# KTH-RPL/neural_graph_mapping

Hardware: AMD Instinct MI355X
Metric: ray-samples/sec (train step: fwd+loss+bwd+Adam, 4096 rays x 128 samples per GPU) (higher is better)
Workload: dtype f32 via 3xbf16 split, fp32 accumulate (hidden-layer matrix products, forward and backward); everything else f32; 1 GPU; M1: 8 fields x 512 rays x (64 coarse + 64 depth-guided) samples per GPU, Fourier(64,raw)+2x64 MLP, nrgbd compositing, NRGBD intrinsics; fields_per_gpu=8, rays_per_field=512, samples_per_ray=128, ranks_seen=1, spin_up_steps=200, jitter=in-kernel Philox, launch=hipGraph replay

## Files before the change

### include/ngm_hip.h

```cpp
#ifndef NGM_HIP_H
#define NGM_HIP_H

#include <stdint.h>

#ifdef __cplusplus
extern "C" {
#endif

#define NGM_ABI_VERSION 11
#define NGM_MAX_LAYERS 4
#define NGM_NUM_LOSS_SUMS 16

enum ngm_status {
  NGM_OK = 0,
  NGM_E_INVALID = -1,
  NGM_E_UNSUPPORTED = -2,
  NGM_E_WORKSPACE = -3,
  NGM_E_HIP = -4
};

enum ngm_encoding { NGM_ENC_NONE = 0, NGM_ENC_FOURIER = 1, NGM_ENC_NERF = 2, NGM_ENC_PERMUTO = 3, NGM_ENC_TRIPLANE = 4 };
enum ngm_triplane_mode { NGM_TRI_SUM = 0, NGM_TRI_PRODUCT = 1, NGM_TRI_CONCAT = 2 };
enum ngm_skip_mode { NGM_SKIP_NO = 0, NGM_SKIP_ADD = 1, NGM_SKIP_CONCAT = 2 };
enum ngm_matmul_mode { NGM_MATMUL_F32 = 0, NGM_MATMUL_BF16X3 = 1, NGM_MATMUL_AUTO = 2 };
// ... 327 lines not shown
                            int64_t max_verts, int64_t* faces, int64_t max_faces, void* workspace,
                            int64_t workspace_bytes, void* stream);
int ngm_marching_cubes_tables(int8_t* tri_table, int32_t* tri_count);

enum ngm_kernel_id {
  NGM_K_RENDER_FWD = 0,
  NGM_K_STASH_BWD = 1,
  NGM_K_FIELD_BWD = 2,
  NGM_K_GRAD_REDUCE = 3,
  NGM_K_ADAM = 4,
  NGM_K_POINTS_FWD = 5,
  NGM_K_COMPOSITE_FWD = 6,
  NGM_K_COMPOSITE_BWD = 7,
  NGM_K_HASH_GRAD = 8,
  NGM_K_HASH_REDUCE = 9,
  NGM_K_LOSS_REDUCE = 10,
  NGM_K_KNN_ASSIGN = 11,
  NGM_K_KNN_EVAL = 12,
  NGM_K_SAMPLER = 13,
  NGM_K_COUNT = 14
};
int ngm_profile_enable(int32_t on);
int ngm_profile_reset(void);
int ngm_profile_read(int32_t kernel_id, double* total_ms, int64_t* launches);

int ngm_debug_phase_cycles(unsigned long long* out528);
int ngm_debug_fwd_phase_cycles(unsigned long long* out528);

int ngm_debug_last_bwd_variant(void);
int ngm_debug_last_matmul(int which);
int ngm_debug_last_fwd_one_tile(void);
int ngm_debug_last_comp_fused(void);
int ngm_debug_disable_fused_comp(int on);
int ngm_debug_stash_mode(int mode);
int ngm_debug_last_stash_mode(void);

#define NGM_MAX_PEERS 8
typedef struct ngm_peer_exchange {
  int32_t world, rank;
  void* mailbox[NGM_MAX_PEERS];
  unsigned long long* seq;
  int32_t* status;
} ngm_peer_exchange;
int64_t ngm_peer_mailbox_bytes(void);
int ngm_peer_alloc(int64_t bytes, void** ptr);
int ngm_peer_free(void* ptr);
int ngm_ipc_export(void* ptr, unsigned char handle[64]);
int ngm_ipc_open(const unsigned char handle[64], void** ptr);
int ngm_ipc_close(void* ptr);
int ngm_loss_exchange(const ngm_peer_exchange* px, float* loss_sums , void* stream);
double ngm_peer_set_timeout(double seconds);

#ifdef __cplusplus
}
#endif
#endif
```

### neural_graph_mapping_amd/_capi.py

```python
import ctypes as C
import os

HERE = os.path.dirname(os.path.abspath(__file__))
LIB_PATH = os.environ.get("NGM_LIB_PATH") or os.path.join(HERE, "lib", "libngm_hip.so")

NGM_MAX_LAYERS = 4
NGM_NUM_LOSS_SUMS = 16
ENC = {"none": 0, "fourier": 1, "nerf": 2, "permuto": 3, "triplane": 4}
TRI = {"sum": 0, "product": 1, "concat": 2}
SCALE = {"no": 0, "unit_ball": 1, "unit_cube": 2}
GEO = {"nrgbd": 0, "occupancy": 1, "density": 2, "neus": 3}
PHOTO = {"l1": 0, "l2": 1, "gaussian_nll": 2}
DEPTH = {"huber": 0, "gaussian_nll": 1, "laplacian_nll": 2}
LS = dict(PHOTO_SUM=0, PHOTO_CNT=1, DEPTH_SUM=2, DEPTH_CNT=3, FS_SUM=4, FS_CNT=5, TSDF_SUM=6,
          TSDF_CNT=7, TERM_SUM=8, TERM_CNT=9, PHOTO_L1_SUM=10)

f32p = C.c_void_p
LArr = C.c_void_p * (NGM_MAX_LAYERS + 1)
SArr = C.c_int64 * (NGM_MAX_LAYERS + 1)


class FieldCfg(C.Structure):
    _fields_ = [("encoding", C.c_int32), ("dim_enc", C.c_int32), ("raw_coords", C.c_int32),
                ("num_octaves", C.c_int32), ("start_octave", C.c_int32), ("num_layers", C.c_int32),
# ... 178 lines not shown
    L.ngm_ipc_close.argtypes = [vp]
    L.ngm_loss_exchange.argtypes = [P(PeerExchange), vp, vp]
    L.ngm_peer_set_timeout.argtypes = [C.c_double]
    L.ngm_peer_set_timeout.restype = C.c_double
    L.ngm_adam_sparse_multi.restype = C.c_int
    L.ngm_step_advance.restype = C.c_int
    L.ngm_field_eval_knn.argtypes = [P(FieldCfg), P(Params), i32, i64, vp, vp, vp, i32, f32, f32, f32, vp, vp, i64, vp]
    L.ngm_field_eval_knn_workspace.argtypes = [i32, i64, i32]
    L.ngm_field_eval_knn_workspace.restype = i64
    L.ngm_render_eval_knn.argtypes = [P(FieldCfg), P(RenderCfg), P(Params), i32, vp, vp, P(Rays), i32, f32, f32, f32, i32,
                                      P(Prediction), vp, i64, vp]
    L.ngm_render_eval_knn.restype = C.c_int
    L.ngm_render_eval_knn_workspace.argtypes = [P(RenderCfg), i32, i32, i32]
    L.ngm_render_eval_knn_workspace.restype = i64
    L.ngm_target_visibility.argtypes = [P(Keyframes), i32, vp, i32, vp, f32, vp, vp, vp]
    L.ngm_target_rays.argtypes = [P(Keyframes), i32, i32, vp, f32, vp, vp, vp, P(TargetOut), vp]
    L.ngm_target_visibility.restype = C.c_int
    L.ngm_target_rays.restype = C.c_int
    L.ngm_target_sv_intersect.argtypes = [i32, i64, vp, vp, f32, vp, vp]
    L.ngm_target_sv_intersect.restype = C.c_int
    L.ngm_target_sv_rays.argtypes = [i32, i32, vp, f32, vp, vp, vp, i32, i32, f32, f32, f32, f32, P(TargetOut), vp]
    L.ngm_target_sv_rays.restype = C.c_int
    L.ngm_target_sample_mv_workspace.argtypes = [i32, i32, i32, i32]
    L.ngm_target_sample_mv_workspace.restype = i64
    L.ngm_target_sample_mv.argtypes = [P(Keyframes), P(TargetSample), P(TargetOut), vp, i64, vp]
    L.ngm_target_sample_mv.restype = C.c_int
    L.ngm_marching_cubes_workspace.argtypes = [i32, i32, i32]
    L.ngm_marching_cubes_workspace.restype = i64
    L.ngm_marching_cubes_count.argtypes = [vp, i32, i32, i32, f32, vp, vp, i64, vp]
    L.ngm_marching_cubes_emit.argtypes = [vp, i32, i32, i32, f32, vp, i64, vp, i64, vp, i64, vp]
    L.ngm_marching_cubes_tables.argtypes = [vp, vp]
    for name in ("ngm_marching_cubes_count", "ngm_marching_cubes_emit", "ngm_marching_cubes_tables"):
        getattr(L, name).restype = C.c_int
    L.ngm_profile_enable.argtypes = [i32]
    L.ngm_profile_read.argtypes = [i32, P(C.c_double), P(i64)]
    for name in ("ngm_profile_enable", "ngm_profile_reset", "ngm_profile_read"):
        getattr(L, name).restype = C.c_int
    for name in ("ngm_sample_rays", "ngm_field_eval_fwd", "ngm_field_eval_bwd", "ngm_composite_fwd",
                 "ngm_composite_bwd", "ngm_render_fwd", "ngm_render_bwd", "ngm_render_bwd_seeded",
                 "ngm_render_read_samples", "ngm_adam_sparse", "ngm_field_eval_knn", "ngm_device_info"):
        getattr(L, name).restype = C.c_int
    _lib = L
    return L


EXPORTED = ["ngm_abi_version", "ngm_last_error", "ngm_device_info", "ngm_permuto_fill_scales", "ngm_sample_rays", "ngm_sample_rays_world", "ngm_sample_rays_weighted",
            "ngm_composite_fwd_packed",
            "ngm_field_eval_fwd", "ngm_encode_fwd", "ngm_encode_bwd", "ngm_encode_bwd_workspace", "ngm_field_eval_bwd", "ngm_field_eval_bwd_workspace",
            "ngm_field_eval_stash_bytes", "ngm_field_eval_fwd_train", "ngm_field_eval_bwd_stash",
            "ngm_composite_fwd", "ngm_composite_bwd", "ngm_render_workspace", "ngm_render_fwd",
            "ngm_render_bwd", "ngm_render_bwd_adam", "ngm_render_bwd_seeded", "ngm_render_bwd_seeded_vars", "ngm_render_read_samples", "ngm_adam_sparse",
            "ngm_field_eval_knn", "ngm_field_eval_knn_workspace", "ngm_render_eval_knn", "ngm_render_eval_knn_workspace", "ngm_adam_sparse_multi", "ngm_step_advance", "ngm_profile_enable", "ngm_profile_reset", "ngm_profile_read",
            "ngm_debug_phase_cycles", "ngm_debug_fwd_phase_cycles", "ngm_debug_last_bwd_variant", "ngm_debug_last_matmul", "ngm_debug_last_fwd_one_tile", "ngm_debug_last_comp_fused", "ngm_debug_disable_fused_comp", "ngm_debug_stash_mode", "ngm_debug_last_stash_mode", "ngm_target_visibility", "ngm_target_rays", "ngm_target_sv_intersect", "ngm_target_sv_rays",
            "ngm_target_sample_mv_workspace", "ngm_target_sample_mv",
            "ngm_render_fwd_counted", "ngm_render_bwd_counted", "ngm_render_bwd_adam_counted",
            "ngm_peer_mailbox_bytes", "ngm_peer_alloc", "ngm_peer_free", "ngm_ipc_export", "ngm_ipc_open", "ngm_ipc_close", "ngm_loss_exchange", "ngm_peer_set_timeout",
            "ngm_marching_cubes_workspace", "ngm_marching_cubes_count", "ngm_marching_cubes_emit", "ngm_marching_cubes_tables"]

NO_GRAD_PARAMS = frozenset({"_encoding.random_shift_per_level"})

KERNEL_IDS = dict(render_fwd=0, stash_bwd=1, field_bwd=2, grad_reduce=3, adam=4, points_fwd=5, composite_fwd=6,
                  composite_bwd=7, hash_grad=8, hash_reduce=9, loss_reduce=10, knn_assign=11, knn_eval=12, sampler=13)


NGM_OK, NGM_E_INVALID, NGM_E_UNSUPPORTED, NGM_E_WORKSPACE, NGM_E_HIP = 0, -1, -2, -3, -4


class NgmError(RuntimeError):

    def __init__(self, msg, code=None):
        super().__init__(msg)
        self.code = code


def check(rc, what=""):
    if rc != 0:
        msg = lib().ngm_last_error().decode(errors="replace")
        raise NgmError(f"{what} failed with status {rc}: {msg}", code=int(rc))


SKIP = {"no": 0, "add": 1, "concat": 2}
STASH = {"full": 0, "half": 1}
HASH_ATOMICS = {"exact": 0, "float": 1}
MATMUL = {"f32": 0, "bf16x3": 1, "auto": 2}


# ... 117 lines not shown
```

### neural_graph_mapping_amd/csrc/ngm_api.hip

```cpp
#include <hip/hip_runtime.h>
#include <stdio.h>
#include <stdlib.h>
#include <string.h>

#include "../../include/ngm_hip.h"
#include "ngm_launch.h"

int ngm_launch_sampler_weighted(const ngm_render_cfg* rc, const ngm_rays* rays, int S, int B, const float* boundaries,
                                const float* weights, float* points_cam, float* distances, float* dirs, hipStream_t st);
int ngm_launch_sampler(const ngm_render_cfg* rc, const ngm_rays* rays, int S, float* points_cam, float* distances,
                       float* dirs, float* points_world, hipStream_t st);
int ngm_launch_loss_values(const ngm_render_cfg* rc, const float* sums, float* out, hipStream_t st);
int ngm_launch_loss_reduce(const float* partials, int nblocks, float* sums, uint64_t* counter, hipStream_t st);
int ngm_launch_neus_sd_grad(const float* d_isd_rays, int F, int R, const float* neus_sd, int64_t sd_stride,
                            const int64_t* field_index, float* d_sd, hipStream_t st);
int ngm_launch_read_stash(const float4* sa, const float2* sb, int64_t n, float* geoms, float* dists, hipStream_t st);
int ngm_launch_adam(float* param, float* m, float* v, int64_t stride, const float* grad, int64_t gstride,
                    const int64_t* field_index, int F, int64_t numel, int64_t step, float lr, float beta1, float beta2,
                    float eps, float wd, hipStream_t st);
int ngm_launch_adam_multi(const ngm_adam_tensor* tensors, int n, const int64_t* field_index, int F, int64_t step,
                          const int64_t* step_dev, float lr, float beta1, float beta2, float eps, float wd,
                          int64_t* advance_step, uint64_t* advance_offset, hipStream_t st, const int32_t* num_active = nullptr);
int ngm_launch_step_advance(int64_t* step_dev, uint64_t* off_dev, hipStream_t st);
int64_t ngm_mc_workspace_bytes(int nx, int ny, int nz);
int ngm_launch_mc_count(const float* vol, int nx, int ny, int nz, float iso, int64_t* counts, void* workspace,
                        int64_t workspace_bytes, hipStream_t st);
int ngm_launch_mc_emit(const float* vol, int nx, int ny, int nz, float iso, float* verts, int64_t max_verts,
                       int64_t* faces, int64_t max_faces, void* workspace, int64_t workspace_bytes, hipStream_t st);
int ngm_mc_copy_tables(int8_t* tri_table, int32_t* tri_count);
int ngm_launch_knn(const ngm_field_cfg* fc, const ngm_params* pr, int num_fields, int64_t P, const float* points,
                   const float* pos, const float* quat, int K, float distance_factor, float outside_value, float mask_radius,
                   float* out, void* workspace, int64_t workspace_bytes, hipStream_t st);
int64_t ngm_knn_workspace_bytes(int num_fields, int64_t P, int K);
int64_t ngm_knn_render_workspace_bytes(int num_fields, int ray_block, int S, int K);
int ngm_launch_render_eval_knn(const ngm_field_cfg* fc, const ngm_render_cfg* rc, const ngm_params* pr, int num_fields,
                               const float* pos, const float* quat, const ngm_rays* rays, int K, float distance_factor,
                               float outside_value, float mask_radius, int ray_block, const ngm_prediction* pred,
                               void* workspace, int64_t workspace_bytes, hipStream_t st);

// ... 274 lines not shown
    return fail(NGM_E_INVALID, "ngm_target_sample_mv: NULL output array");
  if ((int64_t)s->capacity * s->num_rays > INT32_MAX) return fail(NGM_E_UNSUPPORTED, "ngm_target_sample_mv: capacity x num_rays >= 2^31");
  const int64_t need = ngm_target_sample_mv_bytes(kf->num_frames, s->num_current, s->num_fields, s->capacity);
  if (!workspace || workspace_bytes < need) return fail(NGM_E_WORKSPACE, "ngm_target_sample_mv: workspace too small");
  ngm_launch_target_sample_mv(*kf, *s, *out, workspace, (hipStream_t)stream);
  return check_launch("ngm_target_sample_mv");
}

int ngm_target_sv_intersect(int32_t F, int64_t N, const float* field_pos_cam, const float* points_cam, float radius, uint8_t* hit,
                            void* stream) {
  if (F < 0 || N < 0 || radius < 0.f || (F > 0 && N > 0 && (!field_pos_cam || !points_cam || !hit)))
    return fail(NGM_E_INVALID, "ngm_target_sv_intersect: bad argument");
  if (F == 0 || N == 0) return NGM_OK;
  if (F > 65535) return fail(NGM_E_UNSUPPORTED, "ngm_target_sv_intersect: more than 65535 candidate fields");
  ngm_launch_target_sv_intersect(F, N, field_pos_cam, points_cam, radius, hit, (hipStream_t)stream);
  return check_launch("ngm_target_sv_intersect");
}
int ngm_target_sv_rays(int32_t F, int32_t R, const float* field_pos_cam, float radius, const int64_t* pts_ijs, const int64_t* segments,
                       const float* image, int32_t height, int32_t width, float fx, float fy, float cx, float cy,
                       const ngm_target_out* out, void* stream) {
  if (F < 0 || R < 1 || height < 1 || width < 1 || !field_pos_cam || !pts_ijs || !segments || !image || !out || !out->ijs || !out->near ||
      !out->far || !out->gt || !out->rgbds || !out->rgb_mask || !out->depth_mask || !out->term_probs || !out->term_mask)
    return fail(NGM_E_INVALID, "ngm_target_sv_rays: bad argument");
  if (F == 0) return NGM_OK;
  ngm_launch_target_sv_rays(F, R, field_pos_cam, radius, pts_ijs, segments, image, height, width, fx, fy, cx, cy, *out, (hipStream_t)stream);
  return check_launch("ngm_target_sv_rays");
}

int ngm_debug_last_bwd_variant(void) { return g_last_bwd_variant; }
int ngm_debug_last_matmul(int which) { return (which >= 0 && which < 3) ? g_ngm_last_matmul[which] : -1; }
int ngm_debug_last_fwd_one_tile(void) { return g_ngm_last_fwd_one_tile; }
int ngm_debug_last_comp_fused(void) { return g_last_comp_fused; }
int ngm_debug_disable_fused_comp(int on) { const int old = g_no_fused_comp; g_no_fused_comp = on ? 1 : 0; return old; }

static unsigned long long* g_debug_cycles_fwd = nullptr;
int ngm_debug_fwd_phase_cycles(unsigned long long* out528) {
  if (!g_debug_cycles_fwd || !out528) return NGM_E_INVALID;
  (void)hipDeviceSynchronize();
  return hipMemcpy(out528, g_debug_cycles_fwd, NGM_FWD_DEBUG_WORDS * 8, hipMemcpyDeviceToHost) == hipSuccess ? NGM_OK : NGM_E_HIP;
}
int ngm_debug_phase_cycles(unsigned long long* out528) {
  if (!g_debug_cycles || !out528) return NGM_E_INVALID;
  (void)hipDeviceSynchronize();
  return hipMemcpy(out528, g_debug_cycles, NGM_FWD_DEBUG_WORDS * 8, hipMemcpyDeviceToHost) == hipSuccess ? NGM_OK : NGM_E_HIP;
}

int ngm_device_info(int* ncu, char* name, int name_len) {
  int dev = 0;
  hipDeviceProp_t prop;
  if (hipGetDevice(&dev) != hipSuccess || hipGetDeviceProperties(&prop, dev) != hipSuccess) {
    (void)hipGetLastError();
    return fail(NGM_E_HIP, "no HIP device");
  }
  if (ncu) *ncu = prop.multiProcessorCount;
  if (name && name_len > 0) snprintf(name, name_len, "%s (%s)", prop.name, prop.gcnArchName);
  return NGM_OK;
}

int ngm_sample_rays(const ngm_render_cfg* cfg, const ngm_rays* rays, float* points_cam, float* distances, float* dirs,
                    void* stream) {
  if (!cfg || !rays || !rays->ijs) return fail(NGM_E_INVALID, "ngm_sample_rays: NULL argument");
  const int S = cfg->num_samples_coarse + (rays->gt ? cfg->num_samples_guided : 0);
  if (S < 1) return fail(NGM_E_INVALID, "no samples");
  ngm_launch_sampler(cfg, rays, S, points_cam, distances, dirs, nullptr, (hipStream_t)stream);
  return check_launch("ngm_sample_rays");
}
// ... 923 lines not shown
```

### neural_graph_mapping_amd/csrc/ngm_bwd_b3.h

```cpp
#pragma once
#include "ngm_bwd16.h"

#define B3B_WAVES 4
#define B3B_THREADS 256
#define HT 2048
#define PLANE_G 512

template <int L, bool EG, bool HS = false>
struct LdsB3b {
  static_assert(!HS || L == 2, "half stash: two hidden layers");
  static constexpr int NPL = (L - 1) + (EG ? 1 : 0) + (HS ? 1 : 0);
  static constexpr int plane_slot(int l) { return EG ? l : l - 1; }
  static constexpr int fwd_slot() { return NPL - 1; }
  static constexpr int PLANES = NPL * 3 * PLANE_G * 4 + 512 + 64;
  static constexpr int CONSTS = NPL * 3 * PLANE_G * 4;
  static constexpr int HL = 0;
  static constexpr int H1 = HS ? 0 : HT;
  static constexpr int INB = H1 + ((L == 2) ? HT : 0);
  static constexpr int PB = INB + 768;
  static constexpr int OB = PB + 128;
  static constexpr int INB2 = OB + 128;
  static constexpr int PB2 = INB2 + 768;
  static constexpr int OB2 = PB2 + 128;
  static constexpr int ACCL = OB2 + 128;
  static constexpr int WAVE_TOTAL = ACCL + (HS ? 5 * 256 : 0);
  static constexpr int NT = 4 * L;
  static constexpr int EPI_ACC = B3B_WAVES * NT * 1024;
  static constexpr int EPI = EPI_ACC + B3B_WAVES * (2 * L + 18) * 64;
  static constexpr int BODY = PLANES + B3B_WAVES * WAVE_TOTAL;
  static constexpr int TOTAL = BODY > EPI ? BODY : EPI;
};

__device__ __forceinline__ void issue_tile32(const char* sbase, uint32_t gb, uint32_t n0, uint32_t end, int lane, uint32_t lds_tile) {
#pragma unroll
  for (int k = 0; k < 8; ++k) {
    const uint32_t c = 2 * k + (lane >> 5);
    uint32_t n = n0 + (((uint32_t)lane & 31u) ^ (c & 7u));
    if (n >= end) n = end - 1;
    const uint32_t u = n + gb;
    dma16_so(sbase, (((u >> 5) * 16u + c) * 32u + ((u & 31u) ^ (c & 7u))) * 16u, lds_tile + k * 1024);
  }
}

__device__ __forceinline__ void dma16_x4(const char* sb, uint32_t voff, uint32_t lds_base) {
  uint32_t keep;
  asm volatile(
      "s_mov_b32 %0, m0\n\t"
      "s_mov_b32 m0, %3\n\t"
      "s_nop 0\n\t"
      "global_load_lds_dwordx4 %1, %2 nt\n\t"
      "global_load_lds_dwordx4 %1, %2 offset:1024 nt\n\t"
      "global_load_lds_dwordx4 %1, %2 offset:2048 nt\n\t"
      "global_load_lds_dwordx4 %1, %2 offset:3072 nt\n\t"
      "s_mov_b32 m0, %0"
      : "=&s"(keep)
      : "v"(voff), "s"(sb), "s"(lds_base)
      : "memory");
}
__device__ __forceinline__ void issue_tile32_fast(const char* sbase, uint32_t tile, int lane, uint32_t lds_tile) {
  const char* b0 = sbase + (size_t)__builtin_amdgcn_readfirstlane(tile) * 8192;
  dma16_x4(b0, (uint32_t)lane * 16u, lds_tile);
  dma16_x4(b0 + 4096, (uint32_t)lane * 16u, lds_tile + 4096);
}

struct B3Op { ngm_bf16x8 h, m, l; };
template <int B>
__device__ __forceinline__ B3Op b3_regs(const f32x16& v) {
  float x[8];
#pragma unroll
  for (int e = 0; e < 8; ++e) x[e] = v[8 * B + e];
  B3Op o;
  b3_split8(x, o.h, o.m, o.l);
  return o;
}
template <int B>
__device__ __forceinline__ B3Op b3_regs(const float (&v)[16]) {
  float x[8];
#pragma unroll
  for (int e = 0; e < 8; ++e) x[e] = v[8 * B + e];
  B3Op o;
  b3_split8(x, o.h, o.m, o.l);
  return o;
}
__device__ __forceinline__ B3Op b3_rows(const float4& g0, const float4& g1) {
  const float x[8] = {g0.x, g0.y, g0.z, g0.w, g1.x, g1.y, g1.z, g1.w};
  B3Op o;
  b3_split8(x, o.h, o.m, o.l);
  return o;
}

__device__ __forceinline__ void wgrad_b3_block(const B3Op (&A)[2], const B3Op (&Bx)[2], f32x16 (&acc)[2][2]) {
#define NGM_WG_PRODUCT(PA, PB_)                                                                       \
  _Pragma("unroll") for (int mo = 0; mo < 2; ++mo)                                                    \
    _Pragma("unroll") for (int mi = 0; mi < 2; ++mi) acc[mo][mi] = mfma_bf16(A[mo].PA, Bx[mi].PB_, acc[mo][mi]); \
  __builtin_amdgcn_sched_barrier(0)
  NGM_WG_PRODUCT(l, h);
  NGM_WG_PRODUCT(h, l);
// ... 206 lines not shown
```

### neural_graph_mapping_amd/csrc/ngm_field_bwd_b3.hip

```cpp
#include "ngm_bwd_b3.h"

template <bool NEED_COS, bool ENC_GRAD>
__device__ __forceinline__ void recompute_with_encoding(const ngm_u32x4* __restrict__ P, const float* __restrict__ tile,
                                                        const float* __restrict__ pb, const float4 (&encw)[2], int lane,
                                                        f32x16 (&Hc)[2], float (&Eb)[2][2][8], float (&Cb)[2][2][8]) {
  const int hi = lane >> 5;
  const float inv2pi = 0.15915494309189535f;
  const f32x16 zero = {0.f, 0.f, 0.f, 0.f, 0.f, 0.f, 0.f, 0.f, 0.f, 0.f, 0.f, 0.f, 0.f, 0.f, 0.f, 0.f};
  RowRegs R;
  PlaneRegs W[2];
  float4 pq[2][4];
  load_rows(tile, lane, R);
  load_planes(P, 0, lane, W[0]);
  auto ldq = [&](int q) __attribute__((always_inline)) {
#pragma unroll
    for (int j = 0; j < 4; ++j) {
      const int b = q >> 1, e = 4 * (q & 1) + j;
      pq[q & 1][j] = *reinterpret_cast<const float4*>(pb + 4 * (8 * ((8 * b + e) >> 2) + 4 * hi + (e & 3)));
    }
  };
  ldq(0);
  __builtin_amdgcn_sched_barrier(0);
  B3Op A = b3_rows(R.g[0][0], R.g[0][1]);
  __builtin_amdgcn_sched_barrier(0);
// ... 93 lines not shown
    for (int q = 0; q < 5; ++q) accl[64 * q] = make_float4(0.f, 0.f, 0.f, 0.f);
  }

  f32x16 acc[L][2][2];
#pragma unroll
  for (int l = 0; l < L; ++l)
#pragma unroll
    for (int mo = 0; mo < 2; ++mo)
#pragma unroll
      for (int mi = 0; mi < 2; ++mi)
#pragma unroll
        for (int r = 0; r < 16; ++r) acc[l][mo][mi][r] = 0.f;
  float dbh[L][2], dwo[2][4], dwf[2][3], dbo[4];
#pragma unroll
  for (int m = 0; m < 2; ++m) {
#pragma unroll
    for (int l = 0; l < L; ++l) dbh[l][m] = 0.f;
#pragma unroll
    for (int c = 0; c < 4; ++c) dwo[m][c] = 0.f;
    dwf[m][0] = dwf[m][1] = dwf[m][2] = 0.f;
  }
  dbo[0] = dbo[1] = dbo[2] = dbo[3] = 0.f;

  const uint32_t beg = (uint32_t)chunk * (uint32_t)a.per_block, bend = (uint32_t)min(a.P, (int64_t)beg + a.per_block);
  constexpr uint32_t TSTRIDE = 32 * B3B_WAVES;
  uint32_t first, end, ntiles;
  int32_t tstep;
  if constexpr (FC) {
    const uint32_t wr = (uint32_t)a.per_block / B3B_WAVES, wb = min(bend, beg + (uint32_t)wave * wr);
    end = min(bend, wb + wr);
    ntiles = (end - wb + 31u) >> 5;
    first = wb + 32u * (ntiles - 1u);
    tstep = -32;
  } else {
    end = bend;
    first = beg + 32u * (uint32_t)wave;
    ntiles = first < end ? (end - first + TSTRIDE - 1u) / TSTRIDE : 0u;
    tstep = (int32_t)TSTRIDE;
  }
  FieldStreams fs;
  const bool pts = !FC && a.points != nullptr;
  const char* pts_base = pts ? reinterpret_cast<const char*>(a.points + (int64_t)f * a.P * 3) : nullptr;
  __shared__ float s_pose[12];
  if (pts && threadIdx.x == 0) {
    float div, off;
    scale_consts(a.fc.scale_mode, a.fc.field_radius, &div, &off);
    const bool posed = a.pos != nullptr;
    s_pose[0] = posed ? a.pos[3 * f] : 0.f; s_pose[1] = posed ? a.pos[3 * f + 1] : 0.f; s_pose[2] = posed ? a.pos[3 * f + 2] : 0.f;
    s_pose[3] = posed ? a.quat[4 * f] : 1.f; s_pose[4] = posed ? a.quat[4 * f + 1] : 0.f; s_pose[5] = posed ? a.quat[4 * f + 2] : 0.f;
    s_pose[6] = posed ? a.quat[4 * f + 3] : 0.f; s_pose[7] = div; s_pose[8] = off; s_pose[9] = posed ? 1.f : 0.f;
  }
  {
    const int64_t g0 = (int64_t)f * a.P;
    fs.raytab = pts ? nullptr : reinterpret_cast<const char*>(a.raytab) + 32 * (g0 / a.S);
    fs.dout = reinterpret_cast<const char*>(a.d_out + g0);
    fs.tpair = pts ? nullptr : reinterpret_cast<const char*>(a.stashB + (g0 & ~(int64_t)1));
    fs.par = (uint32_t)(g0 & 1);
    fs.gb = (uint32_t)(g0 & 31);
    fs.act[0] = reinterpret_cast<const char*>(a.act + (g0 >> 5) * 2048);
    fs.act[1] = reinterpret_cast<const char*>(a.act + a.act_layer_stride + (g0 >> 5) * 2048);
  }
  const char* seeds = FC ? reinterpret_cast<const char*>(a.rayseed) + 32 * (((int64_t)f * a.P) / a.S) : nullptr;
  const float inv_s = 1.0f / (float)a.S;
  auto issue_small = [&](uint32_t n0, int which) __attribute__((always_inline)) {
    const uint32_t dst = wl_lds + (which ? LY::INB2 : LY::INB) * 4;
    issue_inputs(fs, a.S, n0, end, lane, dst);
// ... 95 lines not shown
    if (threadIdx.x == 0) {
      const float n_m = s_sums[NGM_LS_PHOTO_CNT], n_d = s_sums[NGM_LS_DEPTH_CNT], n_t = s_sums[NGM_LS_TERM_CNT],
                  n_fs = s_sums[NGM_LS_FS_CNT], n_ts = s_sums[NGM_LS_TSDF_CNT];
      float k_photo = n_m > 0 ? a.rc.w_photometric / (3.0f * n_m) : 0.f;
      if (a.rc.photometric_mode == NGM_PHOTO_L2) k_photo = 2.0f * k_photo;
      s_k[0] = k_photo;
      s_k[1] = n_d > 0 ? a.rc.w_depth / n_d : 0.f;
      s_k[2] = n_t > 0 ? a.rc.w_termination * 2.0f / n_t : 0.f;
      s_k[3] = n_fs > 0 ? a.rc.w_freespace * 2.0f / n_fs : 0.f;
      s_k[4] = n_ts > 0 ? a.rc.w_tsdf * 2.0f / n_ts : 0.f;
      if (blockIdx.x == 0) {
        if (a.loss_partials && a.counter) *a.counter += 1ull;
        if (a.loss_out) loss_values_from_sums(a.rc, s_sums, a.loss_out);
      }
    }
    __syncthreads();
  }
  PTK(3);
  float carryQ = 0.f;
  if constexpr (FC) {
    if (ntiles) carryQ = comp_suffix_beyond(a, (int64_t)f * a.P, end, lane, inv_s, s_k[0], s_k[1], s_k[2]);
  }

  int col[4];
#pragma unroll
  for (int j = 0; j < 4; ++j) col[j] = (i >> 2) * 128 + (i & 3) + 4 * ((4 * hi + j) ^ (i >> 2));
#define COL_OFF(m, r) ((m) * 1024 + col[(r) & 3] + 32 * ((r) >> 2))

  PTK(4);
  DMA_WAIT(0);
  PTK(5);
  TICK_DECL;
  TICK(0);
  for (uint32_t it = 0; it < ntiles; ++it) {
    const uint32_t base = first + (uint32_t)((int32_t)it * tstep);
    const uint32_t nxt = base + (uint32_t)tstep;
    const bool more = it + 1u < ntiles;
    float* HLb = wl + LY::HL;
    float* H1b = wl + LY::H1;
    float* pb_c = pbuf;
    float* ob_c = obuf;
    if constexpr (FC) {
      if (it & 1u) { pb_c = pbuf2; ob_c = obuf2; }
      else {
        const int j = i, h = j >> 4, jj = j & 15;
        const float4* blk = reinterpret_cast<const float4*>(hi ? inb : inb2);
        const float4* in4 = blk + 64 * h;
        const float4 r0 = in4[jj], r1 = in4[16 + jj], dd = in4[32 + jj], sp = in4[48 + jj];
        const float4 q0 = blk[128 + j], q1 = blk[160 + j];
        const uint32_t n = (hi ? base : base - 32u) + (uint32_t)j;
        const bool valid = hi ? (n < end) : more;
        const uint32_t nc = (hi && !valid) ? end - 1 : n;
        const bool odd = ((nc + fs.par) & 1u) != 0u;
        const float t = odd ? sp.z : sp.x, T = odd ? sp.w : sp.y;
        const float x = fmaf(t, r0.w, r0.x), y = fmaf(t, r1.x, r0.y), z = fmaf(t, r1.y, r0.z);
        const float4 kn = *reinterpret_cast<const float4*>(s_k);
        const float k_photo = kn.x, k_depth = kn.y, k_term = kn.z, k_fs = kn.w, k_ts = s_k[4];
        const int rayi = fdiv_idx32((int)nc, inv_s, a.S);
        const int k = (int)nc - rayi * a.S, kr = a.S - 1 - k;
        const float dzc = r1.z, gt = r1.w, geom = dd.w;
        const float dC0 = k_photo * q0.x, dC1 = k_photo * q0.y, dC2 = k_photo * q0.z, dD = k_depth * q0.w, dT = k_term * q1.x;
        const float depth = -(dzc * t);
        float dodg = 0.f;
#ifdef NGM_ABLB_NOCOMP
        {
          WAVE_SYNC();
          *reinterpret_cast<float4*>((hi ? pbuf : pbuf2) + 4 * j) = make_float4(x, y, z, 0.f);
          *reinterpret_cast<float4*>((hi ? obuf : obuf2) + 4 * j) = valid ? dd : make_float4(0.f, 0.f, 0.f, 0.f);
          WAVE_SYNC();
        }
        if (false) {
#else
        {
#endif
        const float occ = occ_pointwise_fast(a.rc.geometry_mode, a.rc.geometry_factor, geom, &dodg);
        const float ak = dC0 * dd.x + dC1 * dd.y + dC2 * dd.z + dD * depth + dT;
        float A = valid ? ak * occ : 0.f, B = valid ? 1.0f - occ : 1.0f;
        const int krv = valid ? kr : 0;
        seg_rscan_affine64(A, B, krv, lane);
        const float Qend = (valid && kr > 63 - lane) ? carryQ : 0.f;
        const float nA = lane_next(A, 0.f), nB = lane_next(B, 1.f);
        const float Qk = (krv >= 1) ? fmaf(nB, Qend, nA) : Qend;
// ... 9 lines not shown
        const float4 dout = valid ? make_float4(cf * w * dC0, cf * w * dC1, cf * w * dC2, dg) : make_float4(0.f, 0.f, 0.f, 0.f);
        WAVE_SYNC();
        *reinterpret_cast<float4*>((hi ? pbuf : pbuf2) + 4 * j) = make_float4(x, y, z, 0.f);
        *reinterpret_cast<float4*>((hi ? obuf : obuf2) + 4 * j) = dout;
        dbo[0] += dout.x; dbo[1] += dout.y; dbo[2] += dout.z; dbo[3] += dout.w;
        WAVE_SYNC();
        }
      }
    } else {
      const int j = i, h = j >> 4, jj = j & 15;
      const float4* in4 = reinterpret_cast<const float4*>(inb) + 64 * h;
      const float4 r0 = in4[jj], r1 = in4[16 + jj], dd = in4[32 + jj], sp = in4[48 + jj];
      const uint32_t n = base + (uint32_t)j;
      const bool valid = n < end;
      const uint32_t nc = valid ? n : end - 1;
      const float t = ((nc + fs.par) & 1u) ? sp.z : sp.x;
      float x = fmaf(t, r0.w, r0.x), y = fmaf(t, r1.x, r0.y), z = fmaf(t, r1.y, r0.z);
      if (pts) {
        const float* pw = inb + 512 + 64 * h + 3 * jj;
        const Vec3 v = scaled_local_point(Vec3{pw[0], pw[1], pw[2]}, s_pose[9] != 0.f, s_pose[0], s_pose[1], s_pose[2], s_pose[3],
                                          s_pose[4], s_pose[5], s_pose[6], s_pose[7], s_pose[8]);
        x = v.x; y = v.y; z = v.z;
      }
      const float4 dout = valid ? dd : make_float4(0.f, 0.f, 0.f, 0.f);
      WAVE_SYNC();
      if (hi == 0) {
        *reinterpret_cast<float4*>(pbuf + 4 * j) = make_float4(x, y, z, 0.f);
        *reinterpret_cast<float4*>(obuf + 4 * j) = dout;
        dbo[0] += dout.x; dbo[1] += dout.y; dbo[2] += dout.z; dbo[3] += dout.w;
      }
      WAVE_SYNC();
    }
    TICK(1);
    f32x16 dY[2], Xc[2];
    float Eb[2][2][8];
    float Cb[2][2][8];
    {
      f32x16 Hc[2];
      const float4 wout[2] = {cwout[i], cwout[32 + i]};
      float4 dOa[2][8];
      if constexpr (HS) {
        const ngm_u32x4* fwdP = planes + LY::fwd_slot() * 3 * PLANE_G;
        {
          const float4 encw[2] = {cenc[i], cenc[32 + i]};
          recompute_with_encoding<NEED_COS, ENC_GRAD>(fwdP, H1b, pb_c, encw, lane, Hc, Eb, Cb);
        }
#pragma unroll
        for (int m = 0; m < 2; ++m)
#pragma unroll
          for (int r = 0; r < 16; ++r) Xc[m][r] = H1b[COL_OFF(m, r)];
#pragma unroll
        for (int e = 0; e < 8; ++e) dOa[0][e] = *reinterpret_cast<const float4*>(ob_c + 4 * (8 * (e >> 2) + 4 * hi + (e & 3)));
        const float b1v[2] = {sm[LY::CONSTS + 512 + i], sm[LY::CONSTS + 512 + 32 + i]};
        {
          const float4 a0 = accl[0], a1 = accl[64];
          const float2 a2 = reinterpret_cast<const float2*>(accl + 128)[0];
          dwo[0][0] = a0.x; dwo[0][1] = a0.y; dwo[0][2] = a0.z; dwo[0][3] = a0.w;
          dwo[1][0] = a1.x; dwo[1][1] = a1.y; dwo[1][2] = a1.z; dwo[1][3] = a1.w;
          dbh[L - 1][0] = a2.x; dbh[L - 1][1] = a2.y;
        }
        __builtin_amdgcn_sched_barrier(0);
#pragma unroll
        for (int m = 0; m < 2; ++m)
#pragma unroll
          for (int r = 0; r < 16; ++r) Hc[m][r] = fmaxf(Hc[m][r] + b1v[m], 0.f);
      } else {
#pragma unroll
        for (int m = 0; m < 2; ++m)
#pragma unroll
// ... 139 lines not shown
    for (int b = 0; b < 2; ++b) {
      const float inv2pi = 0.15915494309189535f;
#pragma unroll
      for (int e = 0; e < 8; ++e) {
        const float4 p = ppa[b][e];
#pragma unroll
        for (int m = 0; m < 2; ++m) {
          const float4 w = encw[m];
#ifdef NGM_ABLB_NOENC
          Eb[b][m][e] = p.x + w.x;
          if (ENC_GRAD) dwf[m][0] += dE[m][8 * b + e];
          continue;
#endif
          const float arg = fmaf(w.z, p.z, fmaf(w.y, p.y, w.x * p.x));
          const float rev = __builtin_amdgcn_fractf(arg * inv2pi);
          const float sn = __builtin_amdgcn_sinf(rev);
          float v = sn;
          if (NEED_COS) v = (w.w == NGM_FK_COS) ? __builtin_amdgcn_cosf(rev) : sn;
          if (m == 0) v = (w.w == NGM_FK_RAW) ? arg : v;
          Eb[b][m][e] = v;
          if (ENC_GRAD) {
            const float g = dE[m][8 * b + e] * __builtin_amdgcn_cosf(rev);
            dwf[m][0] = fmaf(g, p.x, dwf[m][0]); dwf[m][1] = fmaf(g, p.y, dwf[m][1]); dwf[m][2] = fmaf(g, p.z, dwf[m][2]);
          }
        }
      }
      __builtin_amdgcn_sched_barrier(0);
    }
    }
    if constexpr (HS && ENC_GRAD) {
      accl[192] = make_float4(dwf[0][0], dwf[0][1], dwf[0][2], 0.f);
      accl[256] = make_float4(dwf[1][0], dwf[1][1], dwf[1][2], 0.f);
    }
    WAVE_SYNC();
    TICK(3);
    if constexpr (FC) {
      if (it + 2u < ntiles) issue_small(base - 64u, (int)(it & 1u));
    }
    if (more) {
      if constexpr (!FC) {
        if (pts) {
          issue_inputs_pts(fs.dout, pts_base, nxt, end, lane, wl_lds + LY::INB * 4, wl_lds + LY::INB * 4 + 2048);
          issue_inputs_pts(fs.dout, pts_base, nxt + 16, end, lane, wl_lds + LY::INB * 4 + 1024, wl_lds + LY::INB * 4 + 2048 + 256);
        } else {
          issue_inputs(fs, a.S, nxt, end, lane, wl_lds + LY::INB * 4);
          issue_inputs(fs, a.S, nxt + 16, end, lane, wl_lds + LY::INB * 4 + 1024);
        }
      }
      const uint32_t u0 = nxt + fs.gb;
      if (((u0 & 31u) == 0u) && (nxt + 32u <= end)) {
        if constexpr (!HS) issue_tile32_fast(fs.act[L - 1], u0 >> 5, lane, wl_lds + LY::HL * 4);
        if (L == 2) issue_tile32_fast(fs.act[0], u0 >> 5, lane, wl_lds + LY::H1 * 4);
      } else {
        if constexpr (!HS) issue_tile32(fs.act[L - 1], fs.gb, nxt, end, lane, wl_lds + LY::HL * 4);
        if (L == 2) issue_tile32(fs.act[0], fs.gb, nxt, end, lane, wl_lds + LY::H1 * 4);
      }
    }
    __builtin_amdgcn_sched_barrier(0);
    TICK(5);
    {
      B3Op A0[2] = {b3_regs<0>(dY[0]), b3_regs<0>(dY[1])}, B0[2] = {b3_arr(Eb[0][0]), b3_arr(Eb[0][1])};
      __builtin_amdgcn_sched_barrier(0);
      B3Op A1[2] = {b3_regs<1>(dY[0]), b3_regs<1>(dY[1])}, B1[2] = {b3_arr(Eb[1][0]), b3_arr(Eb[1][1])};
      wgrad_b3_block_free(A0, B0, acc[0]);
      NGM_INTERLEAVE(24, 8)
      __builtin_amdgcn_sched_barrier(0);
      wgrad_b3_block(A1, B1, acc[0]);
    }
    __builtin_amdgcn_sched_barrier(0);
    TICK(10);
    DMA_WAIT(0);
    TICK(2);
    WAVE_SYNC();
  }
#undef COL_OFF
  PTK(6);
  if constexpr (HS) {
    const float4 a0 = accl[0], a1 = accl[64], a2 = accl[128], f0 = accl[192], f1 = accl[256];
    dwo[0][0] = a0.x; dwo[0][1] = a0.y; dwo[0][2] = a0.z; dwo[0][3] = a0.w;
    dwo[1][0] = a1.x; dwo[1][1] = a1.y; dwo[1][2] = a1.z; dwo[1][3] = a1.w;
    dbh[L - 1][0] = a2.x; dbh[L - 1][1] = a2.y; dbh[0][0] = a2.z; dbh[0][1] = a2.w;
    dwf[0][0] = f0.x; dwf[0][1] = f0.y; dwf[0][2] = f0.z;
    dwf[1][0] = f1.x; dwf[1][1] = f1.y; dwf[1][2] = f1.z;
  }
  __syncthreads();

  float* stage = sm;
  constexpr int NT = LY::NT;
  constexpr int NV = 2 * L + 8 + 6 + 4;
  static_assert(LY::EPI_ACC + B3B_WAVES * NV * 64 <= LY::TOTAL, "the per-feature vectors are staged behind the accumulator tiles");
  float* stagev = sm + LY::EPI_ACC;
#pragma unroll
  for (int l = 0; l < L; ++l)
// ... 163 lines not shown
```

### neural_graph_mapping_amd/csrc/ngm_field_fwd.hip

```cpp
#include "ngm_field.h"
#include "ngm_launch.h"

#include <algorithm>
#include <cstring>

#define WAVE_SYNC()                                        \
  do {                                                     \
    __builtin_amdgcn_fence(__ATOMIC_RELEASE, "wavefront"); \
    __builtin_amdgcn_wave_barrier();                       \
    __builtin_amdgcn_fence(__ATOMIC_ACQUIRE, "wavefront"); \
  } while (0)

template <int MI, int MH, int L, bool NEED_COS, int HASH, int SKIP, bool B3 = false, int NT = NGM_BLOCK>
__global__ __launch_bounds__(NT) void k_field_points_fwd(PointsFwdArgs a) {
  extern __shared__ __attribute__((aligned(16))) float sm[];
  const int f = blockIdx.x % a.F, chunk = blockIdx.x / a.F;
  const int64_t row = a.pr.field_index ? a.pr.field_index[f] : f;
  {
    FieldStage<MI, MH, L, SKIP == 2> fstage;
    fstage.issue(a.fc, a.pr, row);
    fstage.commit(sm, a.fc);
  }
  __syncthreads();
  ngm_u32x4* const b3w = reinterpret_cast<ngm_u32x4*>(sm + FieldLds<MI, MH, L, SKIP == 2>::TOTAL);
  if constexpr (B3) {
    b3_build_planes<MI, MH, L>(sm, b3w);
    __syncthreads();
  }
  const int lane = threadIdx.x & 63, wave = threadIdx.x >> 6;
  float div, off;
  scale_consts(a.fc.scale_mode, a.fc.field_radius, &div, &off);
  const bool posed = a.pos != nullptr;
  float px = 0, py = 0, pz = 0, qw = 1, qx = 0, qy = 0, qz = 0;
  if (posed) {
// ... 541 lines not shown
          const float p0 = tg.x - ra[0], p1 = tg.y - ra[1], p2 = tg.z - ra[2];
          const float l1 = fabsf(p0) + fabsf(p1) + fabsf(p2);
          if (a.rc.photometric_mode == NGM_PHOTO_GAUSSIAN_NLL) {
            ls[NGM_LS_PHOTO_SUM] += (0.5f * p0 * p0 / ra[5] + logf(sqrtf(ra[5]))) + (0.5f * p1 * p1 / ra[6] + logf(sqrtf(ra[6]))) +
                                    (0.5f * p2 * p2 / ra[7] + logf(sqrtf(ra[7])));
            ls[NGM_LS_PHOTO_L1_SUM] += l1;
          } else
            ls[NGM_LS_PHOTO_SUM] += (a.rc.photometric_mode == NGM_PHOTO_L2) ? fmaf(p2, p2, fmaf(p1, p1, p0 * p0))
                                                                             : l1;
          cnt_r += 1u;
          const float e = ra[3] - tg.w, ae = fabsf(e), dlt = a.rc.huber_delta;
          if (a.rc.depth_mode == NGM_DEPTH_GAUSSIAN_NLL) {
            const float dv = ra[8] + 1e-15f;
            ls[NGM_LS_DEPTH_SUM] += 0.5f * e * e / dv + logf(sqrtf(dv));
          } else if (a.rc.depth_mode == NGM_DEPTH_LAPLACIAN_NLL)
            ls[NGM_LS_DEPTH_SUM] += ae / sqrtf(0.5f * ra[8] + 1e-6f) + 0.5f * logf(2.0f * ra[8] + 1e-6f);
          else
            ls[NGM_LS_DEPTH_SUM] += (ae < dlt) ? 0.5f * e * e : dlt * (ae - 0.5f * dlt);
          cnt_r += 1u << 10;
        }
        if (ra[10] != 0.f) {
          const float e = term - ra[11];
          ls[NGM_LS_TERM_SUM] += e * e; cnt_r += 1u << 20;
        }
        if (a.rayseed) {
          const float e0 = ra[0] - tg.x, e1 = ra[1] - tg.y, e2 = ra[2] - tg.z, ed = ra[3] - tg.w, dlt = a.rc.huber_delta;
          const bool l2 = a.rc.photometric_mode == NGM_PHOTO_L2;
          float4 s0 = make_float4(0.f, 0.f, 0.f, 0.f);
          if (m) {
            s0.x = l2 ? e0 : (float)((e0 > 0.f) - (e0 < 0.f)); s0.y = l2 ? e1 : (float)((e1 > 0.f) - (e1 < 0.f));
            s0.z = l2 ? e2 : (float)((e2 > 0.f) - (e2 < 0.f));
            s0.w = (fabsf(ed) < dlt) ? ed : dlt * (float)((ed > 0.f) - (ed < 0.f));
          }
          float4* o = reinterpret_cast<float4*>(a.rayseed + ray * 8);
          o[0] = s0;
          o[1] = make_float4((ra[10] != 0.f) ? term - ra[11] : 0.f, 0.f, 0.f, 0.f);
        }
      }
    }
    WAVE_SYNC();
    PTICK(pc, 10);
    if (rb + BR < r_end) prepare(rb + BR);
  }
  if (a.has_targets && a.loss_partials) {
    __syncthreads();
    float* red = sm + LY::TOTAL;
    ls[NGM_LS_FS_CNT] = (float)(cnt_s & 0xffffu); ls[NGM_LS_TSDF_CNT] = (float)(cnt_s >> 16);
    ls[NGM_LS_PHOTO_CNT] = (float)(cnt_r & 1023u); ls[NGM_LS_DEPTH_CNT] = (float)((cnt_r >> 10) & 1023u);
    ls[NGM_LS_TERM_CNT] = (float)(cnt_r >> 20);
#pragma unroll
    for (int i = 0; i < 11; ++i) {
      const float v = wave_sum(ls[i]);
      if (lane == 0) red[wave * 16 + i] = v;
    }
    __syncthreads();
    if (threadIdx.x < NGM_NUM_LOSS_SUMS) {
      float v = 0.f;
      if (threadIdx.x < 11)
        for (int w = 0; w < nwaves; ++w) v += red[w * 16 + threadIdx.x];
      a.loss_partials[(int64_t)blockIdx.x * NGM_NUM_LOSS_SUMS + threadIdx.x] = v;
    }
  }
#ifdef NGM_PHASE_TIMING
  PTICK(pc, 11);
  if (pc && blockIdx.x == gridDim.x / 2 && threadIdx.x == 0) {
    for (int k = 0; k < 14; ++k) a.debug_cycles[k] = pclk.acc[k];
    a.debug_cycles[14] = __builtin_readcyclecounter() - pclk.start;
    a.debug_cycles[15] = __builtin_amdgcn_s_memrealtime() - pclk.rstart;
  }
// ... 150 lines not shown
```

Before: 2.264 billion ray-samples/s.

## Skip dead rays in bf16x3 field backward and rebalance live tiles across waves

The forward compositing kernel now flags rays whose gradient contribution is provably zero (no depth or termination mask, and the first sample lies beyond the truncation band) in a spare rayseed slot. The bf16x3 backward kernel reads these flags: each wave ballots the dead flags to redistribute only live ray tiles evenly across waves, and inside the tile loop it skips the matmul and weight-gradient work and the activation prefetch for dead tiles. This targets wasted backward work on rays that contribute nothing. In exchange it adds a per-wave flag scan and extra branching, and it depends on the deadness predicate being exactly right, otherwise gradients change.

```diff
diff --git a/include/ngm_hip.h b/include/ngm_hip.h
--- a/include/ngm_hip.h
+++ b/include/ngm_hip.h
@@ -383,6 +383,8 @@
 int ngm_debug_last_fwd_one_tile(void);
 int ngm_debug_last_comp_fused(void);
 int ngm_debug_disable_fused_comp(int on);
+int ngm_debug_b3_partition(const uint8_t* dead, int32_t R, int32_t S, int64_t per_block, int32_t blocks_per_field, int32_t* first_tile,
+                           int32_t* num_tiles);
 int ngm_debug_stash_mode(int mode);
 int ngm_debug_last_stash_mode(void);
 
diff --git a/neural_graph_mapping_amd/_capi.py b/neural_graph_mapping_amd/_capi.py
--- a/neural_graph_mapping_amd/_capi.py
+++ b/neural_graph_mapping_amd/_capi.py
@@ -234,6 +234,8 @@
     L.ngm_marching_cubes_tables.argtypes = [vp, vp]
     for name in ("ngm_marching_cubes_count", "ngm_marching_cubes_emit", "ngm_marching_cubes_tables"):
         getattr(L, name).restype = C.c_int
+    L.ngm_debug_b3_partition.argtypes = [vp, i32, i32, i64, i32, vp, vp]
+    L.ngm_debug_b3_partition.restype = C.c_int
     L.ngm_profile_enable.argtypes = [i32]
     L.ngm_profile_read.argtypes = [i32, P(C.c_double), P(i64)]
     for name in ("ngm_profile_enable", "ngm_profile_reset", "ngm_profile_read"):
@@ -253,7 +255,7 @@
             "ngm_composite_fwd", "ngm_composite_bwd", "ngm_render_workspace", "ngm_render_fwd",
             "ngm_render_bwd", "ngm_render_bwd_adam", "ngm_render_bwd_seeded", "ngm_render_bwd_seeded_vars", "ngm_render_read_samples", "ngm_adam_sparse",
             "ngm_field_eval_knn", "ngm_field_eval_knn_workspace", "ngm_render_eval_knn", "ngm_render_eval_knn_workspace", "ngm_adam_sparse_multi", "ngm_step_advance", "ngm_profile_enable", "ngm_profile_reset", "ngm_profile_read",
-            "ngm_debug_phase_cycles", "ngm_debug_fwd_phase_cycles", "ngm_debug_last_bwd_variant", "ngm_debug_last_matmul", "ngm_debug_last_fwd_one_tile", "ngm_debug_last_comp_fused", "ngm_debug_disable_fused_comp", "ngm_debug_stash_mode", "ngm_debug_last_stash_mode", "ngm_target_visibility", "ngm_target_rays", "ngm_target_sv_intersect", "ngm_target_sv_rays",
+            "ngm_debug_phase_cycles", "ngm_debug_fwd_phase_cycles", "ngm_debug_last_bwd_variant", "ngm_debug_last_matmul", "ngm_debug_last_fwd_one_tile", "ngm_debug_last_comp_fused", "ngm_debug_disable_fused_comp", "ngm_debug_b3_partition", "ngm_debug_stash_mode", "ngm_debug_last_stash_mode", "ngm_target_visibility", "ngm_target_rays", "ngm_target_sv_intersect", "ngm_target_sv_rays",
             "ngm_target_sample_mv_workspace", "ngm_target_sample_mv",
             "ngm_render_fwd_counted", "ngm_render_bwd_counted", "ngm_render_bwd_adam_counted",
             "ngm_peer_mailbox_bytes", "ngm_peer_alloc", "ngm_peer_free", "ngm_ipc_export", "ngm_ipc_open", "ngm_ipc_close", "ngm_loss_exchange", "ngm_peer_set_timeout",
diff --git a/neural_graph_mapping_amd/csrc/ngm_api.hip b/neural_graph_mapping_amd/csrc/ngm_api.hip
--- a/neural_graph_mapping_amd/csrc/ngm_api.hip
+++ b/neural_graph_mapping_amd/csrc/ngm_api.hip
@@ -5,6 +5,7 @@
 
 #include "../../include/ngm_hip.h"
 #include "ngm_launch.h"
+#include "ngm_ray_dead.h"
 
 int ngm_launch_sampler_weighted(const ngm_render_cfg* rc, const ngm_rays* rays, int S, int B, const float* boundaries,
                                 const float* weights, float* points_cam, float* distances, float* dirs, hipStream_t st);
@@ -345,6 +346,33 @@
 int ngm_debug_last_fwd_one_tile(void) { return g_ngm_last_fwd_one_tile; }
 int ngm_debug_last_comp_fused(void) { return g_last_comp_fused; }
 int ngm_debug_disable_fused_comp(int on) { const int old = g_no_fused_comp; g_no_fused_comp = on ? 1 : 0; return old; }
+int ngm_debug_b3_partition(const uint8_t* dead, int32_t R, int32_t S, int64_t per_block, int32_t blocks_per_field, int32_t* first_tile,
+                           int32_t* num_tiles) {
+  const int W = NGM_WAVES_PER_BLOCK;
+  if (!dead || !first_tile || !num_tiles || R < 1 || S < 32 || S % 32 || per_block < 32 * W || per_block % (32 * W) || blocks_per_field < 1 ||
+      (int64_t)R * S >= ((int64_t)1 << 24))
+    return fail(NGM_E_INVALID, "ngm_debug_b3_partition: bad argument");
+  const uint32_t P = (uint32_t)R * (uint32_t)S, G = (uint32_t)(W * blocks_per_field), tpr = (uint32_t)S >> 5;
+  std::vector<uint32_t> live_rays;
+  for (int r = 0; r < R; ++r)
+    if (!dead[r]) live_rays.push_back((uint32_t)r);
+  const bool rebalance = ngm_b3_rebalance_ok((uint32_t)R, (uint32_t)S, G) && (int)live_rays.size() < R;
+  for (uint32_t g = 0; g < G; ++g) {
+    uint32_t wb, end;
+    ngm_b3_static_range(P, (uint32_t)per_block, (uint32_t)W, g / W, g % W, &wb, &end);
+    uint32_t t0 = wb >> 5, nt = (end - wb + 31u) >> 5;
+    if (rebalance) {
+      uint32_t lo, hi;
+      ngm_b3_live_range((uint32_t)live_rays.size() * tpr, G, g, &lo, &hi);
+      if (hi > lo) {
+        t0 = ngm_b3_live_tile(live_rays[lo / tpr], lo, tpr);
+        nt = ngm_b3_live_tile(live_rays[(hi - 1u) / tpr], hi - 1u, tpr) - t0 + 1u;
+      } else nt = 0;
+    }
+    first_tile[g] = (int32_t)t0; num_tiles[g] = (int32_t)nt;
+  }
+  return NGM_OK;
+}
 
 static unsigned long long* g_debug_cycles_fwd = nullptr;
 int ngm_debug_fwd_phase_cycles(unsigned long long* out528) {
diff --git a/neural_graph_mapping_amd/csrc/ngm_bwd_b3.h b/neural_graph_mapping_amd/csrc/ngm_bwd_b3.h
--- a/neural_graph_mapping_amd/csrc/ngm_bwd_b3.h
+++ b/neural_graph_mapping_amd/csrc/ngm_bwd_b3.h
@@ -1,5 +1,6 @@
 #pragma once
 #include "ngm_bwd16.h"
+#include "ngm_ray_dead.h"
 
 #define B3B_WAVES 4
 #define B3B_THREADS 256
@@ -63,6 +64,43 @@
   dma16_x4(b0 + 4096, (uint32_t)lane * 16u, lds_tile + 4096);
 }
 
+__device__ __forceinline__ void b3_rebalance(const float* __restrict__ flags, uint32_t R, uint32_t S, uint32_t G, uint32_t g, int lane,
+                                             uint32_t& first, uint32_t& end, uint32_t& ntiles) {
+  float v[NGM_B3_SCAN_LOADS];
+#pragma unroll
+  for (int q = 0; q < NGM_B3_SCAN_LOADS; ++q) {
+    const uint32_t ray = 64u * (uint32_t)q + (uint32_t)lane;
+    v[q] = ray < R ? flags[8 * (size_t)ray] : 1.f;
+  }
+  uint64_t live[NGM_B3_SCAN_LOADS];
+  uint32_t pre[NGM_B3_SCAN_LOADS], nlive = 0;
+#pragma unroll
+  for (int q = 0; q < NGM_B3_SCAN_LOADS; ++q) {
+    live[q] = __builtin_amdgcn_ballot_w64(v[q] == 0.f);
+    pre[q] = nlive;
+    nlive += (uint32_t)__builtin_popcountll(live[q]);
+  }
+  if (nlive == R) return;
+  const uint32_t tpr = S >> 5;
+  uint32_t lo, hi;
+  ngm_b3_live_range(nlive * tpr, G, g, &lo, &hi);
+  if (hi <= lo) { ntiles = 0; return; }
+  const uint64_t below = ((uint64_t)1 << lane) - 1u;
+  auto kth_live_ray = [&](uint32_t k) __attribute__((always_inline)) {
+    uint64_t w = 0;
+    uint32_t p = 0, q0 = 0;
+#pragma unroll
+    for (int q = 0; q < NGM_B3_SCAN_LOADS; ++q)
+      if (k >= pre[q]) { w = live[q]; p = pre[q]; q0 = (uint32_t)q; }
+    const bool mine = ((w >> lane) & 1u) != 0u && p + (uint32_t)__builtin_popcountll(w & below) == k;
+    return 64u * q0 + (uint32_t)__builtin_ctzll(__builtin_amdgcn_ballot_w64(mine));
+  };
+  const uint32_t t0 = ngm_b3_live_tile(kth_live_ray(lo / tpr), lo, tpr), t1 = ngm_b3_live_tile(kth_live_ray((hi - 1u) / tpr), hi - 1u, tpr);
+  end = 32u * (t1 + 1u);
+  ntiles = t1 - t0 + 1u;
+  first = 32u * t1;
+}
+
 struct B3Op { ngm_bf16x8 h, m, l; };
 template <int B>
 __device__ __forceinline__ B3Op b3_regs(const f32x16& v) {
diff --git a/neural_graph_mapping_amd/csrc/ngm_field_bwd_b3.hip b/neural_graph_mapping_amd/csrc/ngm_field_bwd_b3.hip
--- a/neural_graph_mapping_amd/csrc/ngm_field_bwd_b3.hip
+++ b/neural_graph_mapping_amd/csrc/ngm_field_bwd_b3.hip
@@ -149,6 +149,10 @@
     ntiles = (end - wb + 31u) >> 5;
     first = wb + 32u * (ntiles - 1u);
     tstep = -32;
+    const uint32_t R_ = (uint32_t)a.P / (uint32_t)a.S, G_ = (uint32_t)(B3B_WAVES * a.blocks_per_field);
+    if (ngm_b3_rebalance_ok(R_, (uint32_t)a.S, G_))
+      b3_rebalance(a.rayseed + ((int64_t)f * R_) * 8 + NGM_SEED_DEAD_SLOT, R_, (uint32_t)a.S, G_, (uint32_t)(chunk * B3B_WAVES + wave), lane,
+                   first, end, ntiles);
   } else {
     end = bend;
     first = beg + 32u * (uint32_t)wave;
@@ -310,6 +314,18 @@
   PTK(5);
   TICK_DECL;
   TICK(0);
+  const bool skip_ok = FC && (a.S & 31) == 0;
+  bool dead_cur = false, dead_nxt = false;
+  auto issue_act = [&](uint32_t nxt) __attribute__((always_inline)) {
+    const uint32_t u0 = nxt + fs.gb;
+    if (((u0 & 31u) == 0u) && (nxt + 32u <= end)) {
+      if constexpr (!HS) issue_tile32_fast(fs.act[L - 1], u0 >> 5, lane, wl_lds + LY::HL * 4);
+      if (L == 2) issue_tile32_fast(fs.act[0], u0 >> 5, lane, wl_lds + LY::H1 * 4);
+    } else {
+      if constexpr (!HS) issue_tile32(fs.act[L - 1], fs.gb, nxt, end, lane, wl_lds + LY::HL * 4);
+      if (L == 2) issue_tile32(fs.act[0], fs.gb, nxt, end, lane, wl_lds + LY::H1 * 4);
+    }
+  };
   for (uint32_t it = 0; it < ntiles; ++it) {
     const uint32_t base = first + (uint32_t)((int32_t)it * tstep);
     const uint32_t nxt = base + (uint32_t)tstep;
@@ -319,13 +335,18 @@
     float* pb_c = pbuf;
     float* ob_c = obuf;
     if constexpr (FC) {
-      if (it & 1u) { pb_c = pbuf2; ob_c = obuf2; }
-      else {
+      if (it & 1u) {
+        pb_c = pbuf2; ob_c = obuf2;
+        dead_cur = dead_nxt;
+        dead_nxt = skip_ok && more && __builtin_amdgcn_readfirstlane(__builtin_bit_cast(int, inb[512 + 128 + NGM_SEED_DEAD_SLOT - 4])) != 0;
+      } else {
         const int j = i, h = j >> 4, jj = j & 15;
         const float4* blk = reinterpret_cast<const float4*>(hi ? inb : inb2);
         const float4* in4 = blk + 64 * h;
         const float4 r0 = in4[jj], r1 = in4[16 + jj], dd = in4[32 + jj], sp = in4[48 + jj];
         const float4 q0 = blk[128 + j], q1 = blk[160 + j];
+        dead_cur = skip_ok && __builtin_amdgcn_readlane(__builtin_bit_cast(int, q1.y), 32) != 0;
+        dead_nxt = skip_ok && more && __builtin_amdgcn_readlane(__builtin_bit_cast(int, q1.y), 0) != 0;
         const uint32_t n = (hi ? base : base - 32u) + (uint32_t)j;
         const bool valid = hi ? (n < end) : more;
         const uint32_t nc = (hi && !valid) ? end - 1 : n;
@@ -401,9 +422,22 @@
       WAVE_SYNC();
     }
     TICK(1);
+    constexpr bool EARLY_OUT = HS;
+    if constexpr (FC && EARLY_OUT) {
+      if (dead_cur) {
+        WAVE_SYNC();
+        if (it + 2u < ntiles) issue_small(base - 64u, (int)(it & 1u));
+        if (more && !dead_nxt) issue_act(nxt);
+        DMA_WAIT(0);
+        WAVE_SYNC();
+        continue;
+      }
+    }
+    const bool live_cur = !FC || EARLY_OUT || !dead_cur;
     f32x16 dY[2], Xc[2];
     float Eb[2][2][8];
     float Cb[2][2][8];
+    if (live_cur) {
     {
       f32x16 Hc[2];
       const float4 wout[2] = {cwout[i], cwout[32 + i]};
@@ -609,6 +643,7 @@
       accl[192] = make_float4(dwf[0][0], dwf[0][1], dwf[0][2], 0.f);
       accl[256] = make_float4(dwf[1][0], dwf[1][1], dwf[1][2], 0.f);
     }
+    }
     WAVE_SYNC();
     TICK(3);
     if constexpr (FC) {
@@ -624,18 +659,11 @@
           issue_inputs(fs, a.S, nxt + 16, end, lane, wl_lds + LY::INB * 4 + 1024);
         }
       }
-      const uint32_t u0 = nxt + fs.gb;
-      if (((u0 & 31u) == 0u) && (nxt + 32u <= end)) {
-        if constexpr (!HS) issue_tile32_fast(fs.act[L - 1], u0 >> 5, lane, wl_lds + LY::HL * 4);
-        if (L == 2) issue_tile32_fast(fs.act[0], u0 >> 5, lane, wl_lds + LY::H1 * 4);
-      } else {
-        if constexpr (!HS) issue_tile32(fs.act[L - 1], fs.gb, nxt, end, lane, wl_lds + LY::HL * 4);
-        if (L == 2) issue_tile32(fs.act[0], fs.gb, nxt, end, lane, wl_lds + LY::H1 * 4);
-      }
+      if (!FC || !dead_nxt) issue_act(nxt);
     }
     __builtin_amdgcn_sched_barrier(0);
     TICK(5);
-    {
+    if (live_cur) {
       B3Op A0[2] = {b3_regs<0>(dY[0]), b3_regs<0>(dY[1])}, B0[2] = {b3_arr(Eb[0][0]), b3_arr(Eb[0][1])};
       __builtin_amdgcn_sched_barrier(0);
       B3Op A1[2] = {b3_regs<1>(dY[0]), b3_regs<1>(dY[1])}, B1[2] = {b3_arr(Eb[1][0]), b3_arr(Eb[1][1])};
diff --git a/neural_graph_mapping_amd/csrc/ngm_field_fwd.hip b/neural_graph_mapping_amd/csrc/ngm_field_fwd.hip
--- a/neural_graph_mapping_amd/csrc/ngm_field_fwd.hip
+++ b/neural_graph_mapping_amd/csrc/ngm_field_fwd.hip
@@ -1,5 +1,6 @@
 #include "ngm_field.h"
 #include "ngm_launch.h"
+#include "ngm_ray_dead.h"
 
 #include <algorithm>
 #include <cstring>
@@ -607,9 +608,12 @@
             s0.z = l2 ? e2 : (float)((e2 > 0.f) - (e2 < 0.f));
             s0.w = (fabsf(ed) < dlt) ? ed : dlt * (float)((ed > 0.f) - (ed < 0.f));
           }
+          const bool flag_ok = (S & 31) == 0 && mode != NGM_GEO_NEUS && mode != NGM_GEO_DENSITY &&
+                               a.rc.photometric_mode != NGM_PHOTO_GAUSSIAN_NLL && a.rc.depth_mode == NGM_DEPTH_HUBER;
+          const bool dead = flag_ok && ray_is_dead(ra[9] != 0.f, ra[10] != 0.f && a.rc.w_termination != 0.f, rt[11], wl.tbuf[lane * S], tau);
           float4* o = reinterpret_cast<float4*>(a.rayseed + ray * 8);
           o[0] = s0;
-          o[1] = make_float4((ra[10] != 0.f) ? term - ra[11] : 0.f, 0.f, 0.f, 0.f);
+          o[1] = make_float4((ra[10] != 0.f) ? term - ra[11] : 0.f, dead ? 1.f : 0.f, 0.f, 0.f);
         }
       }
     }
diff --git a/neural_graph_mapping_amd/csrc/ngm_ray_dead.h b/neural_graph_mapping_amd/csrc/ngm_ray_dead.h
--- /dev/null
+++ b/neural_graph_mapping_amd/csrc/ngm_ray_dead.h
@@ -0,0 +1,36 @@
+#pragma once
+#include <stdint.h>
+
+#if !defined(__HIPCC__) && !defined(__host__)
+#define __host__
+#define __device__
+#endif
+
+#define NGM_SEED_DEAD_SLOT 5
+
+__host__ __device__ static inline bool ray_is_dead(bool depth_mask, bool term_active, float gt, float t_min, float tau) {
+  if (depth_mask || term_active) return false;
+  if (!(tau >= 0.0f)) return false;
+  if (gt == 0.0f) return t_min >= 0.0f;
+  return (t_min - gt) >= tau;
+}
+
+__host__ __device__ static inline void ngm_b3_static_range(uint32_t P, uint32_t per_block, uint32_t waves, uint32_t chunk, uint32_t wave,
+                                                           uint32_t* wb, uint32_t* end) {
+  const uint32_t beg = chunk * per_block, bend = P < beg + per_block ? P : beg + per_block;
+  const uint32_t wr = per_block / waves;
+  const uint32_t b = bend < beg + wave * wr ? bend : beg + wave * wr;
+  *wb = b;
+  *end = bend < b + wr ? bend : b + wr;
+}
+__host__ __device__ static inline void ngm_b3_live_range(uint32_t T, uint32_t G, uint32_t g, uint32_t* lo, uint32_t* hi) {
+  *lo = g * T / G;
+  *hi = (g + 1u) * T / G;
+}
+#define NGM_B3_SCAN_LOADS 8
+__host__ __device__ static inline bool ngm_b3_rebalance_ok(uint32_t R, uint32_t S, uint32_t G) {
+  return S != 0u && (S & 31u) == 0u && R <= 64u * NGM_B3_SCAN_LOADS && (uint64_t)R * (S >> 5) * ((uint64_t)G + 1u) < ((uint64_t)1 << 32);
+}
+__host__ __device__ static inline uint32_t ngm_b3_live_tile(uint32_t kth_live_ray, uint32_t j, uint32_t tpr) {
+  return kth_live_ray * tpr + j % tpr;
+}
```

Result: slower. 2.078 billion ray-samples/s (-8.2%).
